# SenseTime-FVG/OpenDWM

Hardware: NVIDIA H100
Metric: CTSD-3.5 6view x 16f denoise-steps/sec (higher is better)
Workload: dtype fp16

## Files before the change

opendwm_b200/csrc/gemm.cu:

```cuda
#include <stdlib.h>
#include <string.h>

#include "gemm_epilogue.cuh"

namespace dwm {

constexpr int STAGES = 4;
constexpr int A_STAGE_BYTES = BM * BK * 2;

template <int NT>
struct GemmCfg {
  static constexpr int kBStageBytes = NT * BK * 2;
  static constexpr int kSmemBytes =
      STAGES * (A_STAGE_BYTES + kBStageBytes) + EPI_STAGE_BYTES + 1024  + 256 ;
};

template <typename TA, typename T, int EPI, int NT, int CL>
__global__ void __launch_bounds__(GEMM_THREADS, 1)
    gemm_wgmma_kernel(const __grid_constant__ CUtensorMap tmap_a,
                      const __grid_constant__ CUtensorMap tmap_b, int M, int N, int K,
                      EpiParams p) {
  constexpr int B_STAGE_BYTES = GemmCfg<NT>::kBStageBytes;
  constexpr int BKE = BK * 2 / static_cast<int>(sizeof(TA));
  extern __shared__ uint8_t smem_raw[];
  uint8_t* smem = smem_raw + ((1024u - (smem_u32(smem_raw) & 1023u)) & 1023u);
  uint8_t* smem_a = smem;
  uint8_t* smem_b = smem + STAGES * A_STAGE_BYTES;
  float* epi_stage = reinterpret_cast<float*>(smem + STAGES * (A_STAGE_BYTES + B_STAGE_BYTES));
  uint64_t* bars = reinterpret_cast<uint64_t*>(smem + STAGES * (A_STAGE_BYTES + B_STAGE_BYTES) + EPI_STAGE_BYTES);
  uint64_t* full_bar = bars;
  uint64_t* empty_bar = bars + STAGES;

  const int warp = threadIdx.x >> 5;
  const int lane = threadIdx.x & 31;
  const int wg = threadIdx.x >> 7;
  const uint32_t rank = CL == 2 ? cluster_ctarank() : 0u;

  const int m_blocks = (M + BM - 1) / BM;
  const int n_blocks = (N + NT - 1) / NT;
  const int k_blocks = (K + BKE - 1) / BKE;
  const int num_tiles = ((m_blocks + CL - 1) / CL) * n_blocks;
  const int first = static_cast<int>(blockIdx.x) / CL, step = static_cast<int>(gridDim.x) / CL;

  if (warp == 0 && lane == 0) {
    tma_prefetch_desc(&tmap_a);
    tma_prefetch_desc(&tmap_b);
    for (int s = 0; s < STAGES; ++s) {
      mbar_init(&full_bar[s], 1);
      mbar_init(&empty_bar[s], CL * EPI_WARPS);
    }
    fence_barrier_init();
  }
  if constexpr (CL == 2) cluster_sync_all(); else __syncthreads();

  if (wg == 0) {
    setmaxnreg_dec<PRODUCER_REGS>();
    if (warp == 0 && elect_one()) {
      int stage = 0;
      uint32_t phase = 0;
      for (int tile = first; tile < num_tiles; tile += step) {
        const int m_blk = (tile / n_blocks) * CL + static_cast<int>(rank);
        const int n_blk = tile % n_blocks;
        for (int kb = 0; kb < k_blocks; ++kb) {
          mbar_wait(&empty_bar[stage], phase ^ 1);
          mbar_expect_tx(&full_bar[stage], A_STAGE_BYTES + B_STAGE_BYTES);
          tma_load_2d(&tmap_a, &full_bar[stage], smem_a + stage * A_STAGE_BYTES, kb * BKE,
                      m_blk * BM, kEvictNormal);
          if constexpr (CL == 2) {
            tma_load_2d_mc(&tmap_b, &full_bar[stage], smem_b + stage * B_STAGE_BYTES + rank * (B_STAGE_BYTES / 2),
                           kb * BKE, n_blk * NT + static_cast<int>(rank) * (NT / 2), 0x3, kEvictLast);
          } else {
            tma_load_2d(&tmap_b, &full_bar[stage], smem_b + stage * B_STAGE_BYTES, kb * BKE,
                        n_blk * NT, kEvictLast);
          }
          if (++stage == STAGES) {
            stage = 0;
            phase ^= 1;
          }
        }
      }
    }
    __syncwarp();
  } else {
    setmaxnreg_inc<CONSUMER_REGS>();
    const int cw = wg - 1;
    const int wrow = cw * 64 + (warp & 3) * 16;
    float* stg = epi_stage + (warp - 4) * 512;
    int stage = 0;
    uint32_t phase = 0;
    for (int tile = first; tile < num_tiles; tile += step) {
      const int m_blk = (tile / n_blocks) * CL + static_cast<int>(rank);
      const int n_blk = tile % n_blocks;
      const int t = threadIdx.x & 127;
      prefetch_resid_tile<EPI, NT>(p, m_blk * BM + cw * 64 + (t >> 1), M, n_blk * NT, N, t & 1);
      float acc[NT / 2];
      wg_mainloop<TA, NT, CL>(acc, smem_a, A_STAGE_BYTES, cw * 64 * 128, smem_b, B_STAGE_BYTES, full_bar,
                              empty_bar, STAGES, k_blocks, stage, phase, lane, rank ^ 1u);
      if constexpr (sizeof(TA) == 1)
        dequant_frag<NT>(acc, p.a_scale, p.w_scale, m_blk * BM + wrow, M, n_blk * NT, N, lane);
      drain_tile<T, EPI, NT>(acc, stg, m_blk * BM, wrow, M, n_blk * NT, N, p, lane);
    }
  }
  if constexpr (CL == 2) cluster_sync_all();
}

int g_resid_tma = 1;

template <typename TA, typename T, int EPI, int NT, int CL>
static int launch_gemm(const dwm_linear_args* a, cudaStream_t stream) {
  constexpr int eb = static_cast<int>(sizeof(TA));
  CUtensorMap ta, tb;
  int rc = make_tmap_2d(&ta, a->A, a->M, a->K, a->lda, BM, BK * 2 / eb, eb);
  if (rc) return rc;
  rc = make_tmap_2d(&tb, a->W, a->N, a->K, a->ldw, NT / CL, BK * 2 / eb, eb);
  if (rc) return rc;

  EpiParams p;
  fill_epi_params(p, a);
  p.resid_prefetch = g_resid_tma;

  constexpr int smem_bytes = GemmCfg<NT>::kSmemBytes;
  auto kern = gemm_wgmma_kernel<TA, T, EPI, NT, CL>;
  static bool attr_set = false;
  if (!attr_set) {
    DWM_CHECK_CUDA(cudaFuncSetAttribute(kern, cudaFuncAttributeMaxDynamicSharedMemorySize, smem_bytes));
    attr_set = true;
  }
  const long long m_blocks = (a->M + BM - 1) / BM;
  const long long n_blocks = (a->N + NT - 1) / NT;
  const long long tiles = ((m_blocks + CL - 1) / CL) * n_blocks;
  const long long slots = sm_count() / CL;
  const int grid = CL * static_cast<int>(tiles < slots ? tiles : slots);
  const int Mi = static_cast<int>(a->M), Ni = static_cast<int>(a->N), Ki = static_cast<int>(a->K);
  if constexpr (CL == 1) {
    kern<<<grid, GEMM_THREADS, smem_bytes, stream>>>(ta, tb, Mi, Ni, Ki, p);
  } else {
    DWM_CHECK_CUDA(launch_cluster2(kern, grid, GEMM_THREADS, smem_bytes, stream,
                                   ta, tb, Mi, Ni, Ki, p));
  }
  DWM_CHECK_CUDA(cudaGetLastError());
  return 0;
}

int g_gemm_bn = 0;
int g_gemm_2cta = -1;

static int pick_tile_n(const dwm_linear_args* a, int cl) {
  if (a->epilogue == DWM_EPI_GEGLU) return 256;
  if (g_gemm_bn == 128 || g_gemm_bn == 256) return g_gemm_bn;
  const long long slots = sm_count() / cl;
  const long long m_groups = ((a->M + BM - 1) / BM + cl - 1) / cl;
  const long long t256 = m_groups * ((a->N + 255) / 256), t128 = m_groups * ((a->N + 127) / 128);
  const long long waves256 = (t256 + slots - 1) / slots, waves128 = (t128 + slots - 1) / slots;
  return waves128 * 128 * 10 < waves256 * 256 * 9 ? 128 : 256;
}

template <typename TA, typename T, int EPI, int CL>
static int launch_pick_n(const dwm_linear_args* a, cudaStream_t s) {
  if (pick_tile_n(a, CL) == 128) return launch_gemm<TA, T, EPI, 128, CL>(a, s);
  return launch_gemm<TA, T, EPI, 256, CL>(a, s);
}

template <typename TA, typename T, int CL, typename TF = T>
static int dispatch_epi(const dwm_linear_args* a, cudaStream_t s) {
  switch (a->epilogue) {
    case DWM_EPI_STORE: return launch_pick_n<TA, T, DWM_EPI_STORE, CL>(a, s);
    case DWM_EPI_GEGLU: return launch_gemm<TA, T, DWM_EPI_GEGLU, 256, CL>(a, s);
    case DWM_EPI_QKNORM: return launch_pick_n<TA, T, DWM_EPI_QKNORM, CL>(a, s);
    case DWM_EPI_RESID: return launch_pick_n<TA, TF, DWM_EPI_RESID, CL>(a, s);
    case DWM_EPI_F32: return launch_pick_n<TA, TF, DWM_EPI_F32, CL>(a, s);
    default: set_last_error("dwm_b200_linear: unknown epilogue %d", a->epilogue); return -1;
  }
}

template <int CL>
static int dispatch_e4m3(const dwm_linear_args* a, cudaStream_t s) {
  if (a->out_dtype == DWM_BF16) return dispatch_epi<__nv_fp8_e4m3, __nv_bfloat16, CL>(a, s);
  return dispatch_epi<__nv_fp8_e4m3, __half, CL, __nv_bfloat16>(a, s);
}

}

namespace dwm { int g_attn_tc = -1; extern int g_ln_staged; extern int g_conv_2cta; extern int g_conv_halo; }

extern "C" int dwm_b200_set_option(const char* name, int value) {
  using namespace dwm;
  DWM_REQUIRE(name != nullptr, "dwm_b200_set_option: null name");
  if (strcmp(name, "attn_tc") == 0) { g_attn_tc = value; return 0; }
  if (strcmp(name, "ln_staged") == 0) { g_ln_staged = value; return 0; }
  if (strcmp(name, "gemm_bn") == 0) { g_gemm_bn = value; return 0; }
  if (strcmp(name, "gemm_2cta") == 0) { g_gemm_2cta = value; return 0; }
  if (strcmp(name, "resid_tma") == 0) { g_resid_tma = value; return 0; }
  if (strcmp(name, "conv_2cta") == 0) { g_conv_2cta = value; return 0; }
  if (strcmp(name, "conv_halo") == 0) { g_conv_halo = value; return 0; }
  set_last_error("dwm_b200_set_option: unknown option %s", name);
  return -1;
}

extern "C" int dwm_b200_linear(const dwm_linear_args* a, dwm_stream_t stream) {
  using namespace dwm;
  DWM_REQUIRE(a != nullptr, "dwm_b200_linear: null args");
  DWM_REQUIRE(a->M > 0 && a->N > 0 && a->K > 0, "dwm_b200_linear: empty problem %lld x %lld x %lld",
              (long long)a->M, (long long)a->N, (long long)a->K);
  DWM_REQUIRE(a->M < (1ll << 31) && a->N < (1ll << 31) && a->K < (1ll << 31),
              "dwm_b200_linear: dimension exceeds int32");
  DWM_REQUIRE(a->A && a->W && a->out, "dwm_b200_linear: null A/W/out");
  DWM_REQUIRE(a->K % 8 == 0 && a->lda % 8 == 0 && a->ldw % 8 == 0,
              "dwm_b200_linear: K, lda, ldw must be multiples of 8 (16-byte TMA pitch); got %lld %lld %lld",
              (long long)a->K, (long long)a->lda, (long long)a->ldw);
  if (a->dtype == DWM_E4M3) {
    DWM_REQUIRE(a->K % 16 == 0 && a->lda % 16 == 0 && a->ldw % 16 == 0,
                "dwm_b200_linear: E4M3 needs K, lda, ldw multiples of 16 (16-byte TMA pitch); got %lld %lld %lld",
                (long long)a->K, (long long)a->lda, (long long)a->ldw);
    DWM_REQUIRE(a->a_scale && a->w_scale, "dwm_b200_linear: E4M3 operands need a_scale and w_scale");
    DWM_REQUIRE(a->out_dtype == DWM_BF16 || a->out_dtype == DWM_F16,
                "dwm_b200_linear: E4M3 operands need out_dtype DWM_BF16 or DWM_F16, got %d", a->out_dtype);
    DWM_REQUIRE((reinterpret_cast<uintptr_t>(a->w_scale) & 7) == 0,
                "dwm_b200_linear: w_scale must be 8-byte aligned");
  }
  DWM_REQUIRE((reinterpret_cast<uintptr_t>(a->A) & 15) == 0 &&
                  (reinterpret_cast<uintptr_t>(a->W) & 15) == 0 &&
                  (reinterpret_cast<uintptr_t>(a->out) & 15) == 0,
              "dwm_b200_linear: A, W, out must be 16-byte aligned");
  DWM_REQUIRE(a->N % 32 == 0, "dwm_b200_linear: N must be a multiple of 32, got %lld", (long long)a->N);
  DWM_REQUIRE(a->ldo % 8 == 0, "dwm_b200_linear: ldo must be a multiple of 8");
  if (a->epilogue == DWM_EPI_GEGLU)
    DWM_REQUIRE(a->N % 256 == 0, "dwm_b200_linear: GEGLU needs N %% 256 == 0 (packed weight)");
  if (a->epilogue == DWM_EPI_QKNORM) {
    DWM_REQUIRE(a->N % 64 == 0 && a->qk_region > 0 && a->qk_region % 64 == 0 && a->q_norm_weight &&
                    (a->k_norm_weight || a->qk_norm_regions == 1),
                "dwm_b200_linear: QKNORM needs head_dim 64 regions and both norm weights");
  }
  DWM_REQUIRE(a->n_peer_out >= 0 && a->n_peer_out <= 8, "dwm_b200_linear: n_peer_out out of range");
  if (a->n_peer_out > 0)
    DWM_REQUIRE(a->epilogue == DWM_EPI_STORE || a->epilogue == DWM_EPI_QKNORM || a->epilogue == DWM_EPI_GEGLU,
                "dwm_b200_linear: peer_out needs a 16-bit epilogue");
  if (a->epilogue == DWM_EPI_RESID && a->blend_x)
    DWM_REQUIRE(a->alpha != nullptr, "dwm_b200_linear: blend_x without alpha");
  for (const void* p : {static_cast<const void*>(a->bias), static_cast<const void*>(a->resid),
                        static_cast<const void*>(a->gate), static_cast<const void*>(a->blend_x)})
    DWM_REQUIRE((reinterpret_cast<uintptr_t>(p) & 15) == 0,
                "dwm_b200_linear: bias, resid, gate, blend_x must be 16-byte aligned");
  for (int i = 0; i < a->n_peer_out; ++i)
    DWM_REQUIRE(a->peer_out[i] && (reinterpret_cast<uintptr_t>(a->peer_out[i]) & 15) == 0,
                "dwm_b200_linear: peer_out[%d] must be a 16-byte aligned pointer", i);
  DWM_REQUIRE((!a->resid || a->ldr % 4 == 0) && (!a->gate || a->gate_ld % 4 == 0) &&
                  (!a->blend_x || a->ldx % 4 == 0),
              "dwm_b200_linear: ldr, gate_ld, ldx must be multiples of 4 (16-byte rows); got %lld %lld %lld",
              (long long)a->ldr, (long long)a->gate_ld, (long long)a->ldx);
  if (a->rows_per_item > 0 && a->epilogue != DWM_EPI_RESID && a->epilogue != DWM_EPI_F32)
    DWM_REQUIRE(a->out_item_stride >= a->rows_per_item,
                "dwm_b200_linear: out_item_stride %lld < rows_per_item %lld would write several items "
                "to the same output rows", (long long)a->out_item_stride, (long long)a->rows_per_item);
  cudaStream_t s = reinterpret_cast<cudaStream_t>(stream);
  if (g_gemm_2cta < 0) {
    const char* e = getenv("DWM_GEMM_2CTA");
    g_gemm_2cta = (e && e[0] == '0') ? 0 : 1;
  }
  const bool pair = g_gemm_2cta == 1 && a->M >= 512;
  if (a->dtype == DWM_BF16)
    return pair ? dispatch_epi<__nv_bfloat16, __nv_bfloat16, 2>(a, s) : dispatch_epi<__nv_bfloat16, __nv_bfloat16, 1>(a, s);
  if (a->dtype == DWM_F16) return pair ? dispatch_epi<__half, __half, 2>(a, s) : dispatch_epi<__half, __half, 1>(a, s);
  if (a->dtype == DWM_E4M3) return pair ? dispatch_e4m3<2>(a, s) : dispatch_e4m3<1>(a, s);
  set_last_error("dwm_b200_linear: dtype must be DWM_BF16, DWM_F16 or DWM_E4M3, got %d", a->dtype);
  return -1;
}
```

opendwm_b200/csrc/gemm_epilogue.cuh:

```cuda
#pragma once
#include "common.cuh"
#include "wgmma.cuh"
#include "../../include/dwm_b200.h"

namespace dwm {

constexpr int BM = 128;
constexpr int BK = 64;
constexpr int WG_K = 16;
constexpr int CONSUMER_WGS = 2;
constexpr int GEMM_THREADS = 128 * (1 + CONSUMER_WGS);
constexpr int EPI_WARPS = 4 * CONSUMER_WGS;
constexpr int EPI_STAGE_BYTES = EPI_WARPS * 16 * 32 * 4;
constexpr int PRODUCER_REGS = 40;
constexpr int CONSUMER_REGS = 232;

struct EpiParams {
  void* out;
  long long ldo;
  const float* bias;
  int act;
  long long rows_per_item, out_item_stride, out_row_offset;
  const float* qw;
  const float* kw;
  long long qk_region;
  float eps;
  int norm_regions;
  const float* resid;
  long long ldr, resid_row_mod;
  const float* gate;
  long long gate_ld;
  const float* blend_x;
  long long ldx;
  const float* alpha;
  long long rows_per_batch;
  void* peer_out[8];
  int n_peers;
  int resid_prefetch;
  const float* a_scale;
  const float* w_scale;
};

__device__ __forceinline__ float apply_act(float v, int act) {
  switch (act) {
    case DWM_ACT_GELU_TANH: return gelu_tanh(v);
    case DWM_ACT_GELU_ERF: return gelu_erf(v);
    case DWM_ACT_SILU: return silu(v);
    case DWM_ACT_RELU: return fmaxf(v, 0.f);
    default: return v;
  }
}

__device__ __forceinline__ float resid_elem(float acc, float b, float g, float r) {
  return __fmaf_rn(__fadd_rn(acc, b), g, r);
}
__device__ __forceinline__ float blend_elem(float a, float a1, float x, float v) {
  return __fmaf_rn(a, x, __fmul_rn(a1, v));
}

__device__ __forceinline__ void st_global_v4(void* p, uint32_t a, uint32_t b, uint32_t c,
                                             uint32_t d) {
  asm volatile("st.global.v4.b32 [%0], {%1, %2, %3, %4};" ::"l"(p), "r"(a), "r"(b), "r"(c), "r"(d)
               : "memory");
}


template <int NA>
__device__ __forceinline__ void frag_chunk(const float (&acc)[NA], int c, float (&v)[16]) {
#pragma unroll
  for (int i = 0; i < 16; ++i) v[i] = acc[16 * c + i];
}

__device__ __forceinline__ void stage_dump(float* stg, int lane, const float (&v)[16]) {
  __syncwarp();
  const int r0 = lane >> 2, q0 = (lane & 3) >> 1, h = (lane & 1) * 2;
#pragma unroll
  for (int jj = 0; jj < 4; ++jj) {
    const int q = (2 * jj + q0) ^ r0;
    *reinterpret_cast<float2*>(stg + r0 * 32 + q * 4 + h) = make_float2(v[4 * jj], v[4 * jj + 1]);
    *reinterpret_cast<float2*>(stg + (r0 + 8) * 32 + q * 4 + h) = make_float2(v[4 * jj + 2], v[4 * jj + 3]);
  }
  __syncwarp();
}

__device__ __forceinline__ int frag_col(int lane, int jj, int e) { return 8 * jj + 2 * (lane & 3) + (e & 1); }

struct TileGeom {
  int bw;
  int rows;
  int w_lim;
  int h_lim;
  int img_w;
};

template <typename T, int EPI, int NT>
__device__ __forceinline__ void drain_tile(const float (&acc)[NT / 2], float* stg, int m_base, int row0, int M,
                                           int n_tile0, int N, const EpiParams& p, int lane,
                                           const TileGeom geom = TileGeom{0, 0, 0, 0, 0}) {
  constexpr bool kOut16 = (EPI == DWM_EPI_STORE || EPI == DWM_EPI_GEGLU || EPI == DWM_EPI_QKNORM);
  const int rs = lane >> 3;
  const int c4 = lane & 7;

  int orow[4];
  int rrow[4];
  int item[4];
  float alpha[4];
  const int rpi = static_cast<int>(p.rows_per_item);
#pragma unroll
  for (int it = 0; it < 4; ++it) {
    int m;
    bool valid;
    if (geom.bw > 0) {
      const int r = row0 + it * 4 + rs;
      const int ph = r / geom.bw, pw = r - ph * geom.bw;
      valid = r < geom.rows && pw < geom.w_lim && ph < geom.h_lim;
      m = m_base + ph * geom.img_w + pw;
    } else {
      m = m_base + row0 + it * 4 + rs;
      valid = m < M;
    }
    if (valid) {
      int o = m;
      if (kOut16) {
        if (rpi > 0) o = (m / rpi) * static_cast<int>(p.out_item_stride) + (m % rpi);
        o += static_cast<int>(p.out_row_offset);
      }
      orow[it] = o;
      if (EPI == DWM_EPI_RESID) {
        item[it] = rpi > 0 ? m / rpi : 0;
        rrow[it] = p.resid_row_mod > 0 ? m % static_cast<int>(p.resid_row_mod)
                   : (p.resid_row_mod < 0 ? item[it] : m);
        alpha[it] = p.blend_x ? __ldg(p.alpha + (p.rows_per_batch > 0 ? m / static_cast<int>(p.rows_per_batch) : 0)) : 0.f;
      }
    } else {
      orow[it] = -1;
    }
  }

  auto stg4 = [&](int r) { return *reinterpret_cast<const float4*>(stg + r * 32 + ((c4 ^ (r & 7)) << 2)); };
  auto flush16 = [&](int ocol) {
#pragma unroll
    for (int it = 0; it < 4; ++it) {
      const float4 v = stg4(it * 4 + rs);
      if (orow[it] >= 0) {
        T* dst = reinterpret_cast<T*>(p.out) + static_cast<long long>(orow[it]) * p.ldo + ocol + c4 * 4;
        uint2 pk;
        pk.x = Cvt<T>::pack2(v.x, v.y);
        pk.y = Cvt<T>::pack2(v.z, v.w);
        *reinterpret_cast<uint2*>(dst) = pk;
        const long long eoff = static_cast<long long>(orow[it]) * p.ldo + ocol + c4 * 4;
        for (int q = 0; q < p.n_peers; ++q)
          *reinterpret_cast<uint2*>(reinterpret_cast<T*>(p.peer_out[q]) + eoff) = pk;
      }
    }
  };
  float4 rq[4], bq[4];
  auto prefetch32 = [&](int ocol) {
    if constexpr (EPI == DWM_EPI_RESID) {
      const int col = ocol + c4 * 4;
#pragma unroll
      for (int it = 0; it < 4; ++it) {
        rq[it] = make_float4(0.f, 0.f, 0.f, 0.f);
        bq[it] = make_float4(0.f, 0.f, 0.f, 0.f);
        if (orow[it] >= 0) {
          if (p.resid) rq[it] = *reinterpret_cast<const float4*>(p.resid + static_cast<long long>(rrow[it]) * p.ldr + col);
          if (p.blend_x) bq[it] = *reinterpret_cast<const float4*>(p.blend_x + static_cast<long long>(orow[it]) * p.ldx + col);
        }
      }
    }
  };
  auto flush32 = [&](int ocol) {
    const int col = ocol + c4 * 4;
    float4 b = make_float4(0.f, 0.f, 0.f, 0.f);
    if (EPI == DWM_EPI_RESID && p.bias) b = __ldg(reinterpret_cast<const float4*>(p.bias + col));
#pragma unroll
    for (int it = 0; it < 4; ++it) {
      float4 v = stg4(it * 4 + rs);
      if (orow[it] >= 0) {
        if (EPI == DWM_EPI_RESID) {
          float4 g = make_float4(1.f, 1.f, 1.f, 1.f);
          if (p.gate)
            g = __ldg(reinterpret_cast<const float4*>(p.gate + static_cast<long long>(item[it]) * p.gate_ld + col));
          v.x = resid_elem(v.x, b.x, g.x, rq[it].x); v.y = resid_elem(v.y, b.y, g.y, rq[it].y);
          v.z = resid_elem(v.z, b.z, g.z, rq[it].z); v.w = resid_elem(v.w, b.w, g.w, rq[it].w);
          if (p.blend_x) {
            const float a = alpha[it], a1 = 1.0f - alpha[it];
            v.x = blend_elem(a, a1, bq[it].x, v.x); v.y = blend_elem(a, a1, bq[it].y, v.y);
            v.z = blend_elem(a, a1, bq[it].z, v.z); v.w = blend_elem(a, a1, bq[it].w, v.w);
          }
        }
        *reinterpret_cast<float4*>(reinterpret_cast<float*>(p.out) + static_cast<long long>(orow[it]) * p.ldo + col) = v;
      }
    }
  };

  if constexpr (EPI == DWM_EPI_STORE || EPI == DWM_EPI_F32 || EPI == DWM_EPI_RESID) {
#pragma unroll
    for (int c = 0; c < NT / 32; ++c) {
      const int n0 = n_tile0 + c * 32;
      if (n0 >= N) break;
      prefetch32(n0);
      float v[16];
      frag_chunk(acc, c, v);
      if (EPI != DWM_EPI_RESID) {
        if (p.bias) {
#pragma unroll
          for (int jj = 0; jj < 4; ++jj) {
            const float2 b = __ldg(reinterpret_cast<const float2*>(p.bias + n0 + frag_col(lane, jj, 0)));
            v[4 * jj] += b.x; v[4 * jj + 1] += b.y; v[4 * jj + 2] += b.x; v[4 * jj + 3] += b.y;
          }
        }
        if (p.act == DWM_ACT_GELU_TANH) {
#pragma unroll
          for (int j = 0; j < 16; ++j) v[j] = gelu_tanh(v[j]);
        } else if (p.act == DWM_ACT_SILU) {
#pragma unroll
          for (int j = 0; j < 16; ++j) v[j] = silu(v[j]);
        } else if (p.act == DWM_ACT_GELU_ERF) {
#pragma unroll
          for (int j = 0; j < 16; ++j) v[j] = gelu_erf(v[j]);
        } else if (p.act == DWM_ACT_RELU) {
#pragma unroll
          for (int j = 0; j < 16; ++j) v[j] = fmaxf(v[j], 0.f);
        }
      }
      stage_dump(stg, lane, v);
      if constexpr (EPI == DWM_EPI_STORE) flush16(n0); else flush32(n0);
    }
  } else if constexpr (EPI == DWM_EPI_GEGLU) {
    static_assert(NT == 256, "GEGLU packs value / gate halves per 256-column tile");
#pragma unroll
    for (int c = 0; c < 4; ++c) {
      float a[16], g[16], v[16];
      frag_chunk(acc, c, a);
      frag_chunk(acc, c + 4, g);
      const float* bv = p.bias ? p.bias + n_tile0 + c * 32 : nullptr;
#pragma unroll
      for (int j = 0; j < 16; ++j) {
        float x = a[j], y = g[j];
        if (bv) {
          const int col = frag_col(lane, j >> 2, j);
          x += __ldg(bv + col);
          y += __ldg(bv + 128 + col);
        }
        v[j] = x * gelu_erf(y);
      }
      stage_dump(stg, lane, v);
      flush16(n_tile0 / 2 + c * 32);
    }
  } else {
#pragma unroll
    for (int g = 0; g < NT / 64; ++g) {
      const int n0 = n_tile0 + g * 64;
      if (n0 >= N) break;
      float v0[16], v1[16];
      frag_chunk(acc, 2 * g, v0);
      frag_chunk(acc, 2 * g + 1, v1);
      if (p.bias) {
#pragma unroll
        for (int j = 0; j < 16; ++j) {
          const int col = frag_col(lane, j >> 2, j);
          v0[j] += __ldg(p.bias + n0 + col);
          v1[j] += __ldg(p.bias + n0 + 32 + col);
        }
      }
      const int region = n0 / static_cast<int>(p.qk_region);
      if (region < p.norm_regions) {
        const float* w = region == 0 ? p.qw : p.kw;
        float ss_lo = 0.f, ss_hi = 0.f;
#pragma unroll
        for (int j = 0; j < 16; ++j) {
          if ((j & 3) < 2) ss_lo += v0[j] * v0[j] + v1[j] * v1[j];
          else ss_hi += v0[j] * v0[j] + v1[j] * v1[j];
        }
        ss_lo += __shfl_xor_sync(0xffffffffu, ss_lo, 1);
        ss_lo += __shfl_xor_sync(0xffffffffu, ss_lo, 2);
        ss_hi += __shfl_xor_sync(0xffffffffu, ss_hi, 1);
        ss_hi += __shfl_xor_sync(0xffffffffu, ss_hi, 2);
        const float inv_lo = rsqrtf(ss_lo * (1.0f / 64.0f) + p.eps);
        const float inv_hi = rsqrtf(ss_hi * (1.0f / 64.0f) + p.eps);
#pragma unroll
        for (int j = 0; j < 16; ++j) {
          const int col = frag_col(lane, j >> 2, j);
          const float inv = (j & 3) < 2 ? inv_lo : inv_hi;
          v0[j] = v0[j] * inv * __ldg(w + col);
          v1[j] = v1[j] * inv * __ldg(w + 32 + col);
        }
      }
      stage_dump(stg, lane, v0);
      flush16(n0);
      stage_dump(stg, lane, v1);
      flush16(n0 + 32);
    }
  }
}

template <int NT>
__device__ __forceinline__ void dequant_frag(float (&acc)[NT / 2], const float* a_scale, const float* w_scale,
                                             int m0, int M, int n_tile0, int N, int lane) {
  const int r = m0 + (lane >> 2);
  const float s_lo = r < M ? __ldg(a_scale + r) : 0.f;
  const float s_hi = r + 8 < M ? __ldg(a_scale + r + 8) : 0.f;
#pragma unroll
  for (int g = 0; g < NT / 64; ++g) {
    float2 w[8];
#pragma unroll
    for (int jj = 0; jj < 8; ++jj) {
      const int col = n_tile0 + 8 * (8 * g + jj) + 2 * (lane & 3);
      w[jj] = col < N ? __ldg(reinterpret_cast<const float2*>(w_scale + col)) : make_float2(0.f, 0.f);
    }
#pragma unroll
    for (int jj = 0; jj < 8; ++jj) {
      const int j = 8 * g + jj;
      acc[4 * j + 0] = __fmul_rn(acc[4 * j + 0], __fmul_rn(s_lo, w[jj].x));
      acc[4 * j + 1] = __fmul_rn(acc[4 * j + 1], __fmul_rn(s_lo, w[jj].y));
      acc[4 * j + 2] = __fmul_rn(acc[4 * j + 2], __fmul_rn(s_hi, w[jj].x));
      acc[4 * j + 3] = __fmul_rn(acc[4 * j + 3], __fmul_rn(s_hi, w[jj].y));
    }
    asm volatile("" ::: "memory");
  }
}

template <int NT>
__device__ __forceinline__ void dequant_frag_vol(float (&acc)[NT / 2], float s, const float* w_scale,
                                                 int n_tile0, int N, int lane) {
#pragma unroll
  for (int g = 0; g < NT / 32; ++g) {
    constexpr int G = 4;
    float2 w[G];
#pragma unroll
    for (int jj = 0; jj < G; ++jj) {
      const int col = n_tile0 + 8 * (G * g + jj) + 2 * (lane & 3);
      w[jj] = col < N ? __ldg(reinterpret_cast<const float2*>(w_scale + col)) : make_float2(0.f, 0.f);
    }
#pragma unroll
    for (int jj = 0; jj < G; ++jj) {
      const int j = G * g + jj;
      const float sx = __fmul_rn(s, w[jj].x), sy = __fmul_rn(s, w[jj].y);
      acc[4 * j + 0] = __fmul_rn(acc[4 * j + 0], sx);
      acc[4 * j + 1] = __fmul_rn(acc[4 * j + 1], sy);
      acc[4 * j + 2] = __fmul_rn(acc[4 * j + 2], sx);
      acc[4 * j + 3] = __fmul_rn(acc[4 * j + 3], sy);
    }
    asm volatile("" ::: "memory");
  }
}

template <typename T, int NT, int CL = 1, int TAPS = 1>
__device__ __forceinline__ void wg_mainloop(float (&acc)[NT / 2], const uint8_t* smem_a, int a_stage_bytes,
                                            int a_row_off_bytes, const uint8_t* smem_b, int b_stage_bytes,
                                            uint64_t* full_bar, uint64_t* empty_bar, int stages, int k_iters,
                                            int& stage, uint32_t& phase, int lane, uint32_t peer = 0) {
#pragma unroll
  for (int i = 0; i < NT / 2; ++i) acc[i] = 0.f;
  fence_operands(acc);
  auto release = [&](int s) {
    mbar_arrive(&empty_bar[s]);
    if constexpr (CL == 2) mbar_arrive_remote(mapa_u32(smem_u32(&empty_bar[s]), peer));
  };
  int prev = -1;
  for (int ki = 0; ki < k_iters; ++ki) {
    mbar_wait(&full_bar[stage], phase);
    wgmma_fence();
#pragma unroll
    for (int t = 0; t < TAPS; ++t) {
      const uint64_t da = gmma_desc_sw128(smem_u32(smem_a + stage * a_stage_bytes + a_row_off_bytes + t * 128));
      const uint64_t db = gmma_desc_sw128(smem_u32(smem_b + stage * b_stage_bytes + t * NT * BK * 2));
#pragma unroll
      for (int k = 0; k < BK / WG_K; ++k) Wgmma<NT, T>::ss(acc, da + 2 * k, db + 2 * k, 1u);
    }
    wgmma_commit();
    wgmma_wait<1>();
    if (prev >= 0 && lane == 0) release(prev);
    prev = stage;
    if (++stage == stages) { stage = 0; phase ^= 1; }
  }
  wgmma_wait<0>();
  fence_operands(acc);
  if (prev >= 0 && lane == 0) release(prev);
}

template <int EPI, int NT>
__device__ __forceinline__ void prefetch_resid_tile(const EpiParams& p, int m, int M, int n_tile0,
                                                    int N, int half) {
  constexpr int half_cols = NT / 2;
  if constexpr (EPI == DWM_EPI_RESID) {
    if (!p.resid_prefetch) return;
    const int n0 = n_tile0 + half * half_cols;
    if (m < M && n0 < N) {
      const int cols = (N - n0) < half_cols ? (N - n0) : half_cols;
      const uint32_t bytes = static_cast<uint32_t>(cols) * 4u;
      if (p.resid) {
        if (p.resid_row_mod >= 0) {
          const long long rr = p.resid_row_mod > 0 ? m % static_cast<int>(p.resid_row_mod) : m;
          const float* src = p.resid + rr * p.ldr + n0;
          asm volatile("cp.async.bulk.prefetch.L2.global [%0], %1;" ::"l"(src), "r"(bytes) : "memory");
        }
      }
      if (p.blend_x) {
        const float* src = p.blend_x + static_cast<long long>(m) * p.ldx + n0;
        asm volatile("cp.async.bulk.prefetch.L2.global [%0], %1;" ::"l"(src), "r"(bytes) : "memory");
      }
    }
  }
}

template <typename... KArgs, typename... Args>
inline cudaError_t launch_cluster2(void (*kern)(KArgs...), int grid, int threads, int smem, cudaStream_t s,
                                   Args... args) {
  cudaLaunchConfig_t cfg = {};
  cfg.gridDim = dim3(grid);
  cfg.blockDim = dim3(threads);
  cfg.dynamicSmemBytes = smem;
  cfg.stream = s;
  cudaLaunchAttribute attr[1];
  attr[0].id = cudaLaunchAttributeClusterDimension;
  attr[0].val.clusterDim.x = 2;
  attr[0].val.clusterDim.y = 1;
  attr[0].val.clusterDim.z = 1;
  cfg.attrs = attr;
  cfg.numAttrs = 1;
  return cudaLaunchKernelEx(&cfg, kern, args...);
}

inline void fill_epi_params(EpiParams& p, const dwm_linear_args* a) {
  p.out = a->out;
  p.ldo = a->ldo;
  p.bias = a->bias;
  p.act = a->act;
  p.rows_per_item = a->rows_per_item;
  p.out_item_stride = a->out_item_stride;
  p.out_row_offset = a->out_row_offset;
  p.qw = a->q_norm_weight;
  p.kw = a->k_norm_weight;
  p.qk_region = a->qk_region;
  p.eps = a->eps;
  p.norm_regions = a->qk_norm_regions > 0 ? a->qk_norm_regions : 2;
  p.resid = a->resid;
  p.ldr = a->ldr;
  p.resid_row_mod = a->resid_row_mod;
  p.gate = a->gate;
  p.gate_ld = a->gate_ld;
  p.blend_x = a->blend_x;
  p.ldx = a->ldx;
  p.alpha = a->alpha;
  p.rows_per_batch = a->rows_per_batch;
  p.n_peers = a->n_peer_out;
  p.resid_prefetch = 1;
  for (int i = 0; i < 8; ++i) p.peer_out[i] = i < a->n_peer_out ? a->peer_out[i] : nullptr;
  p.a_scale = a->a_scale;
  p.w_scale = a->w_scale;
}

}
```

Measured before the change: 1.162.

## Add ping-pong WGMMA GEMM kernel alternating consumer warpgroups across tiles

Adds a ping-pong GEMM kernel in which each of the two consumer warpgroups computes a full 128x128 tile (two 64-row wgmma halves), and the two alternate tiles through named barriers. This lets one warpgroup's epilogue overlap the other's mainloop. It uses a 6-stage smem ring and handles GEGLU with 128-wide tiles through remapped weight rows and bias offsets. It is enabled by default for fp16/bf16 when there are many tiles per SM and K<=2048. The risks are higher register pressure, since each consumer holds 128 accumulators, and subtle stage/phase bookkeeping between the alternating warpgroups.

```diff
diff --git a/opendwm_b200/csrc/gemm.cu b/opendwm_b200/csrc/gemm.cu
--- a/opendwm_b200/csrc/gemm.cu
+++ b/opendwm_b200/csrc/gemm.cu
@@ -92,13 +92,134 @@
       const int m_blk = (tile / n_blocks) * CL + static_cast<int>(rank);
       const int n_blk = tile % n_blocks;
       const int t = threadIdx.x & 127;
-      prefetch_resid_tile<EPI, NT>(p, m_blk * BM + cw * 64 + (t >> 1), M, n_blk * NT, N, t & 1);
+      prefetch_resid_tile<EPI, NT / 2>(p, m_blk * BM + cw * 64 + (t >> 1), M, n_blk * NT + (t & 1) * (NT / 2), N);
       float acc[NT / 2];
       wg_mainloop<TA, NT, CL>(acc, smem_a, A_STAGE_BYTES, cw * 64 * 128, smem_b, B_STAGE_BYTES, full_bar,
                               empty_bar, STAGES, k_blocks, stage, phase, lane, rank ^ 1u);
       if constexpr (sizeof(TA) == 1)
         dequant_frag<NT>(acc, p.a_scale, p.w_scale, m_blk * BM + wrow, M, n_blk * NT, N, lane);
       drain_tile<T, EPI, NT>(acc, stg, m_blk * BM, wrow, M, n_blk * NT, N, p, lane);
+    }
+  }
+  if constexpr (CL == 2) cluster_sync_all();
+}
+
+constexpr int PP_NT = 128;
+constexpr int PP_STAGES = 6;
+constexpr int PP_B_STAGE_BYTES = PP_NT * BK * 2;
+constexpr int PP_SMEM_BYTES =
+    PP_STAGES * (A_STAGE_BYTES + PP_B_STAGE_BYTES) + EPI_STAGE_BYTES + 1024  + 256 ;
+static_assert(PP_SMEM_BYTES <= 227 * 1024, "ping-pong ring exceeds shared memory");
+
+template <int EPI>
+__device__ __forceinline__ int pp_w_row(int n_blk, int h) {
+  if constexpr (EPI == DWM_EPI_GEGLU) return (n_blk >> 1) * 256 + (n_blk & 1) * 64 + h * 128;
+  return n_blk * PP_NT + h * 64;
+}
+
+__device__ __forceinline__ void named_bar_sync(int id, int threads) {
+  asm volatile("bar.sync %0, %1;" ::"r"(id), "r"(threads) : "memory");
+}
+__device__ __forceinline__ void named_bar_arrive(int id, int threads) {
+  asm volatile("bar.arrive %0, %1;" ::"r"(id), "r"(threads) : "memory");
+}
+
+template <typename T, int EPI, int CL>
+__global__ void __launch_bounds__(GEMM_THREADS, 1)
+    gemm_pingpong_kernel(const __grid_constant__ CUtensorMap tmap_a,
+                         const __grid_constant__ CUtensorMap tmap_b, int M, int N, int K,
+                         EpiParams p) {
+  extern __shared__ uint8_t smem_raw[];
+  uint8_t* smem = smem_raw + ((1024u - (smem_u32(smem_raw) & 1023u)) & 1023u);
+  uint8_t* smem_a = smem;
+  uint8_t* smem_b = smem + PP_STAGES * A_STAGE_BYTES;
+  float* epi_stage = reinterpret_cast<float*>(smem + PP_STAGES * (A_STAGE_BYTES + PP_B_STAGE_BYTES));
+  uint64_t* bars = reinterpret_cast<uint64_t*>(smem + PP_STAGES * (A_STAGE_BYTES + PP_B_STAGE_BYTES) + EPI_STAGE_BYTES);
+  uint64_t* full_bar = bars;
+  uint64_t* empty_bar = bars + PP_STAGES;
+
+  const int warp = threadIdx.x >> 5;
+  const int lane = threadIdx.x & 31;
+  const int wg = threadIdx.x >> 7;
+  const uint32_t rank = CL == 2 ? cluster_ctarank() : 0u;
+
+  const int m_blocks = (M + BM - 1) / BM;
+  const int n_blocks = (N + PP_NT - 1) / PP_NT;
+  const int k_blocks = (K + BK - 1) / BK;
+  const int num_tiles = ((m_blocks + CL - 1) / CL) * n_blocks;
+  const int first = static_cast<int>(blockIdx.x) / CL, step = static_cast<int>(gridDim.x) / CL;
+
+  if (warp == 0 && lane == 0) {
+    tma_prefetch_desc(&tmap_a);
+    tma_prefetch_desc(&tmap_b);
+    for (int s = 0; s < PP_STAGES; ++s) {
+      mbar_init(&full_bar[s], 1);
+      mbar_init(&empty_bar[s], CL * 4);
+    }
+    fence_barrier_init();
+  }
+  if constexpr (CL == 2) cluster_sync_all(); else __syncthreads();
+
+  if (wg == 0) {
+    setmaxnreg_dec<PRODUCER_REGS>();
+    if (warp == 0 && elect_one()) {
+      int stage = 0;
+      uint32_t phase = 0;
+      for (int tile = first; tile < num_tiles; tile += step) {
+        const int m_blk = (tile / n_blocks) * CL + static_cast<int>(rank);
+        const int n_blk = tile % n_blocks;
+        for (int kb = 0; kb < k_blocks; ++kb) {
+          mbar_wait(&empty_bar[stage], phase ^ 1);
+          mbar_expect_tx(&full_bar[stage], A_STAGE_BYTES + PP_B_STAGE_BYTES);
+          tma_load_2d(&tmap_a, &full_bar[stage], smem_a + stage * A_STAGE_BYTES, kb * BK, m_blk * BM,
+                      kEvictNormal);
+          uint8_t* b = smem_b + stage * PP_B_STAGE_BYTES;
+          if constexpr (CL == 2) {
+            tma_load_2d_mc(&tmap_b, &full_bar[stage], b + rank * (PP_B_STAGE_BYTES / 2), kb * BK,
+                           pp_w_row<EPI>(n_blk, static_cast<int>(rank)), 0x3, kEvictLast);
+          } else {
+            for (int h = 0; h < 2; ++h)
+              tma_load_2d(&tmap_b, &full_bar[stage], b + h * (PP_B_STAGE_BYTES / 2), kb * BK,
+                          pp_w_row<EPI>(n_blk, h), kEvictLast);
+          }
+          if (++stage == PP_STAGES) {
+            stage = 0;
+            phase ^= 1;
+          }
+        }
+      }
+    }
+    __syncwarp();
+  } else {
+    setmaxnreg_inc<CONSUMER_REGS>();
+    const int cw = wg - 1;
+    const int t = threadIdx.x & 127;
+    float* stg = epi_stage + (warp - 4) * 512;
+    const int n_local = first < num_tiles ? (num_tiles - first + step - 1) / step : 0;
+    int stage = 0;
+    uint32_t phase = 0;
+    auto skip = [&](int n) {
+      stage += n;
+      phase ^= static_cast<uint32_t>(stage / PP_STAGES) & 1u;
+      stage %= PP_STAGES;
+    };
+    if (cw == 1) skip(k_blocks);
+    for (int j = cw; j < n_local; j += 2) {
+      const int tile = first + j * step;
+      const int m_blk = (tile / n_blocks) * CL + static_cast<int>(rank);
+      const int n_blk = tile % n_blocks;
+      prefetch_resid_tile<EPI, PP_NT>(p, m_blk * BM + t, M, n_blk * PP_NT, N);
+      if (j > 0) named_bar_sync(1 + cw, 256);
+      const bool pass = j + 1 < n_local;
+      float acc[PP_NT];
+      wg_mainloop<T, PP_NT, CL, 1, 2>(acc, smem_a, A_STAGE_BYTES, 0, smem_b, PP_B_STAGE_BYTES, full_bar,
+                                      empty_bar, PP_STAGES, k_blocks, stage, phase, lane, rank ^ 1u,
+                                      [&] { if (pass) named_bar_arrive(2 - cw, 256); });
+      skip(k_blocks);
+#pragma unroll
+      for (int h = 0; h < 2; ++h)
+        drain_tile<T, EPI, PP_NT>(acc_rows<PP_NT / 2>(acc, h), stg, m_blk * BM, h * 64 + (warp & 3) * 16, M,
+                                  n_blk * PP_NT, N, p, lane);
     }
   }
   if constexpr (CL == 2) cluster_sync_all();
@@ -142,6 +263,39 @@
   return 0;
 }
 
+template <typename T, int EPI, int CL>
+static int launch_pingpong(const dwm_linear_args* a, cudaStream_t stream) {
+  CUtensorMap ta, tb;
+  int rc = make_tmap_2d(&ta, a->A, a->M, a->K, a->lda, BM, BK, 2);
+  if (rc) return rc;
+  rc = make_tmap_2d(&tb, a->W, a->N, a->K, a->ldw, PP_NT / 2, BK, 2);
+  if (rc) return rc;
+
+  EpiParams p;
+  fill_epi_params(p, a);
+  p.resid_prefetch = g_resid_tma;
+
+  auto kern = gemm_pingpong_kernel<T, EPI, CL>;
+  static bool attr_set = false;
+  if (!attr_set) {
+    DWM_CHECK_CUDA(cudaFuncSetAttribute(kern, cudaFuncAttributeMaxDynamicSharedMemorySize, PP_SMEM_BYTES));
+    attr_set = true;
+  }
+  const long long m_blocks = (a->M + BM - 1) / BM;
+  const long long n_blocks = (a->N + PP_NT - 1) / PP_NT;
+  const long long tiles = ((m_blocks + CL - 1) / CL) * n_blocks;
+  const long long slots = sm_count() / CL;
+  const int grid = CL * static_cast<int>(tiles < slots ? tiles : slots);
+  const int Mi = static_cast<int>(a->M), Ni = static_cast<int>(a->N), Ki = static_cast<int>(a->K);
+  if constexpr (CL == 1) {
+    kern<<<grid, GEMM_THREADS, PP_SMEM_BYTES, stream>>>(ta, tb, Mi, Ni, Ki, p);
+  } else {
+    DWM_CHECK_CUDA(launch_cluster2(kern, grid, GEMM_THREADS, PP_SMEM_BYTES, stream, ta, tb, Mi, Ni, Ki, p));
+  }
+  DWM_CHECK_CUDA(cudaGetLastError());
+  return 0;
+}
+
 int g_gemm_bn = 0;
 int g_gemm_2cta = -1;
 
@@ -155,8 +309,25 @@
   return waves128 * 128 * 10 < waves256 * 256 * 9 ? 128 : 256;
 }
 
+int g_gemm_pingpong = -1;
+
+static bool use_pingpong(const dwm_linear_args* a, int cl) {
+  if (g_gemm_pingpong < 0) {
+    const char* e = getenv("DWM_GEMM_PINGPONG");
+    g_gemm_pingpong = e ? atoi(e) : 1;
+  }
+  if (g_gemm_pingpong == 0 || g_gemm_bn != 0 || a->dtype == DWM_E4M3) return false;
+  if (g_gemm_pingpong == 2) return true;
+  const long long slots = sm_count() / cl;
+  const long long tiles = (((a->M + BM - 1) / BM + cl - 1) / cl) * ((a->N + PP_NT - 1) / PP_NT);
+  return tiles >= 16 * slots && a->K <= 2048;
+}
+
 template <typename TA, typename T, int EPI, int CL>
 static int launch_pick_n(const dwm_linear_args* a, cudaStream_t s) {
+  if constexpr (sizeof(TA) == 2) {
+    if (use_pingpong(a, CL)) return launch_pingpong<T, EPI, CL>(a, s);
+  }
   if (pick_tile_n(a, CL) == 128) return launch_gemm<TA, T, EPI, 128, CL>(a, s);
   return launch_gemm<TA, T, EPI, 256, CL>(a, s);
 }
@@ -165,7 +336,11 @@
 static int dispatch_epi(const dwm_linear_args* a, cudaStream_t s) {
   switch (a->epilogue) {
     case DWM_EPI_STORE: return launch_pick_n<TA, T, DWM_EPI_STORE, CL>(a, s);
-    case DWM_EPI_GEGLU: return launch_gemm<TA, T, DWM_EPI_GEGLU, 256, CL>(a, s);
+    case DWM_EPI_GEGLU:
+      if constexpr (sizeof(TA) == 2) {
+        if (use_pingpong(a, CL)) return launch_pingpong<T, DWM_EPI_GEGLU, CL>(a, s);
+      }
+      return launch_gemm<TA, T, DWM_EPI_GEGLU, 256, CL>(a, s);
     case DWM_EPI_QKNORM: return launch_pick_n<TA, T, DWM_EPI_QKNORM, CL>(a, s);
     case DWM_EPI_RESID: return launch_pick_n<TA, TF, DWM_EPI_RESID, CL>(a, s);
     case DWM_EPI_F32: return launch_pick_n<TA, TF, DWM_EPI_F32, CL>(a, s);
@@ -190,6 +365,7 @@
   if (strcmp(name, "ln_staged") == 0) { g_ln_staged = value; return 0; }
   if (strcmp(name, "gemm_bn") == 0) { g_gemm_bn = value; return 0; }
   if (strcmp(name, "gemm_2cta") == 0) { g_gemm_2cta = value; return 0; }
+  if (strcmp(name, "gemm_pingpong") == 0) { g_gemm_pingpong = value; return 0; }
   if (strcmp(name, "resid_tma") == 0) { g_resid_tma = value; return 0; }
   if (strcmp(name, "conv_2cta") == 0) { g_conv_2cta = value; return 0; }
   if (strcmp(name, "conv_halo") == 0) { g_conv_halo = value; return 0; }
diff --git a/opendwm_b200/csrc/gemm_epilogue.cuh b/opendwm_b200/csrc/gemm_epilogue.cuh
--- a/opendwm_b200/csrc/gemm_epilogue.cuh
+++ b/opendwm_b200/csrc/gemm_epilogue.cuh
@@ -228,13 +228,14 @@
       if constexpr (EPI == DWM_EPI_STORE) flush16(n0); else flush32(n0);
     }
   } else if constexpr (EPI == DWM_EPI_GEGLU) {
-    static_assert(NT == 256, "GEGLU packs value / gate halves per 256-column tile");
-#pragma unroll
-    for (int c = 0; c < 4; ++c) {
+    static_assert(NT == 256 || NT == 128, "GEGLU packs value / gate halves per 256-column block");
+    const int wv = (n_tile0 & ~255) + (n_tile0 & 255) / 2;
+#pragma unroll
+    for (int c = 0; c < NT / 64; ++c) {
       float a[16], g[16], v[16];
       frag_chunk(acc, c, a);
-      frag_chunk(acc, c + 4, g);
-      const float* bv = p.bias ? p.bias + n_tile0 + c * 32 : nullptr;
+      frag_chunk(acc, c + NT / 64, g);
+      const float* bv = p.bias ? p.bias + wv + c * 32 : nullptr;
 #pragma unroll
       for (int j = 0; j < 16; ++j) {
         float x = a[j], y = g[j];
@@ -346,13 +347,23 @@
   }
 }
 
-template <typename T, int NT, int CL = 1, int TAPS = 1>
-__device__ __forceinline__ void wg_mainloop(float (&acc)[NT / 2], const uint8_t* smem_a, int a_stage_bytes,
+template <int N, int L>
+__device__ __forceinline__ float (&acc_rows(float (&acc)[L], int h))[N] {
+  return *reinterpret_cast<float(*)[N]>(&acc[h * N]);
+}
+
+struct NoOp {
+  __device__ void operator()() const {}
+};
+
+template <typename T, int NT, int CL = 1, int TAPS = 1, int MW = 1, typename F = NoOp>
+__device__ __forceinline__ void wg_mainloop(float (&acc)[MW * NT / 2], const uint8_t* smem_a, int a_stage_bytes,
                                             int a_row_off_bytes, const uint8_t* smem_b, int b_stage_bytes,
                                             uint64_t* full_bar, uint64_t* empty_bar, int stages, int k_iters,
-                                            int& stage, uint32_t& phase, int lane, uint32_t peer = 0) {
-#pragma unroll
-  for (int i = 0; i < NT / 2; ++i) acc[i] = 0.f;
+                                            int& stage, uint32_t& phase, int lane, uint32_t peer = 0,
+                                            F issued = F{}) {
+#pragma unroll
+  for (int i = 0; i < MW * NT / 2; ++i) acc[i] = 0.f;
   fence_operands(acc);
   auto release = [&](int s) {
     mbar_arrive(&empty_bar[s]);
@@ -364,10 +375,16 @@
     wgmma_fence();
 #pragma unroll
     for (int t = 0; t < TAPS; ++t) {
-      const uint64_t da = gmma_desc_sw128(smem_u32(smem_a + stage * a_stage_bytes + a_row_off_bytes + t * 128));
       const uint64_t db = gmma_desc_sw128(smem_u32(smem_b + stage * b_stage_bytes + t * NT * BK * 2));
-#pragma unroll
-      for (int k = 0; k < BK / WG_K; ++k) Wgmma<NT, T>::ss(acc, da + 2 * k, db + 2 * k, 1u);
+      uint64_t da[MW];
+#pragma unroll
+      for (int h = 0; h < MW; ++h)
+        da[h] = gmma_desc_sw128(smem_u32(smem_a + stage * a_stage_bytes + a_row_off_bytes + h * 64 * 128 + t * 128));
+#pragma unroll
+      for (int k = 0; k < BK / WG_K; ++k) {
+#pragma unroll
+        for (int h = 0; h < MW; ++h) Wgmma<NT, T>::ss(acc_rows<NT / 2>(acc, h), da[h] + 2 * k, db + 2 * k, 1u);
+      }
     }
     wgmma_commit();
     wgmma_wait<1>();
@@ -375,20 +392,18 @@
     prev = stage;
     if (++stage == stages) { stage = 0; phase ^= 1; }
   }
+  issued();
   wgmma_wait<0>();
   fence_operands(acc);
   if (prev >= 0 && lane == 0) release(prev);
 }
 
-template <int EPI, int NT>
-__device__ __forceinline__ void prefetch_resid_tile(const EpiParams& p, int m, int M, int n_tile0,
-                                                    int N, int half) {
-  constexpr int half_cols = NT / 2;
+template <int EPI, int COLS>
+__device__ __forceinline__ void prefetch_resid_tile(const EpiParams& p, int m, int M, int n0, int N) {
   if constexpr (EPI == DWM_EPI_RESID) {
     if (!p.resid_prefetch) return;
-    const int n0 = n_tile0 + half * half_cols;
     if (m < M && n0 < N) {
-      const int cols = (N - n0) < half_cols ? (N - n0) : half_cols;
+      const int cols = (N - n0) < COLS ? (N - n0) : COLS;
       const uint32_t bytes = static_cast<uint32_t>(cols) * 4u;
       if (p.resid) {
         if (p.resid_row_mod >= 0) {
```

Result: faster. 1.177 (median of 6 runs) (+1.3%).
